# luizirber/sourmash-rust

Hardware: AMD Instinct MI355X
Metric: k-mers hashed/sec (k=31, scaled=1000) (higher is better)
Workload: dtype u64

## Files before the change

### sourmash-rust_amd/csrc/sketch_kernels.hip

```cpp
#include <hip/hip_runtime.h>
#include <stdint.h>

#include <cstdio>
#include <cstdlib>
#include <type_traits>

#include "device.hpp"
#include "kernels.hpp"

namespace smh {
namespace {

constexpr uint64_t kC1 = 0x87c37b91114253d5ULL;
constexpr uint64_t kC2 = 0x4cf5ad432745937fULL;

__device__ __forceinline__ uint64_t rotl64(uint64_t x, int r) { return (x << r) | (x >> (64 - r)); }
__device__ __forceinline__ uint64_t fmix64(uint64_t k) {
  k ^= k >> 33;
  k *= 0xff51afd7ed558ccdULL;
  k ^= k >> 33;
  k *= 0xc4ceb9fe1a85ec53ULL;
  k ^= k >> 33;
  return k;
}
// ... 20 lines not shown
    uint32_t r = n & 15u;
    if (r < 8) k1 |= (uint64_t)b << (8 * r);
    else k2 |= (uint64_t)b << (8 * (r - 8));
    n++;
    if ((n & 15u) == 0) { mm3_block(h1, h2, k1, k2); k1 = 0; k2 = 0; }
  }
  __device__ __forceinline__ uint64_t finish() {
    uint32_t rem = n & 15u;
    if (rem > 8) h2 ^= mix_k2(k2);
    if (rem > 0) h1 ^= mix_k1(k1);
    return mm3_finish(h1, h2, n);
  }
};

__device__ __forceinline__ void emit(const CandSink& sink, uint64_t h, uint64_t pos) {
  unsigned long long idx = atomicAdd(sink.count, 1ull);
  if (idx < sink.capacity) {
    sink.hash[idx] = h;
    if (sink.pos) sink.pos[idx] = pos;
  }
}

struct Stage {
  uint32_t* ctl;
  uint64_t* hash;
  uint64_t* pos;
  uint32_t cap;
};
__device__ __forceinline__ void stage_emit(const Stage& st, const CandSink& sink, uint64_t h, uint64_t pos) {
  const uint32_t slot = atomicAdd(&st.ctl[0], 1u);
  if (slot < st.cap) { st.hash[slot] = h; if (sink.pos) st.pos[slot] = pos; }
  else emit(sink, h, pos);
}
__device__ __forceinline__ void stage_flush(const Stage& st, const CandSink& sink, int tid, int nthreads,
                                            uint32_t at_least = 0) {
  __syncthreads();
  const uint32_t staged = min(st.ctl[0], st.cap);
  if (staged && staged >= at_least) {
    if (tid == 0) {
      unsigned long long base = atomicAdd(sink.count, (unsigned long long)staged);
      st.ctl[2] = (uint32_t)base; st.ctl[3] = (uint32_t)(base >> 32);
    }
    __syncthreads();
    const uint64_t base = ((uint64_t)st.ctl[3] << 32) | st.ctl[2];
    for (uint32_t e = tid; e < staged; e += nthreads)
      if (base + e < sink.capacity) {
        sink.hash[base + e] = st.hash[e];
        if (sink.pos) sink.pos[base + e] = st.pos[e];
      }
    __syncthreads();
    if (tid == 0) st.ctl[0] = 0;
  }
}

__device__ __forceinline__ uint32_t find_record(const uint64_t* __restrict__ starts, uint32_t nrec,
                                                uint64_t p) {
  uint32_t lo = 0, hi = nrec;
  while (hi - lo > 1) {
    uint32_t mid = (lo + hi) >> 1;
    if (starts[mid] <= p) lo = mid; else hi = mid;
  }
  return lo;
}

__device__ __forceinline__ uint64_t record_valid_end(const uint64_t* __restrict__ starts, const uint64_t* __restrict__ vends,
                                                     uint32_t min_len, uint32_t r) {
  if (vends) return vends[r];
  const uint64_t s0 = starts[r], s1 = starts[r + 1];
  return (min_len && s1 - s0 < min_len) ? s0 : s1;
}
__global__ __launch_bounds__(256) void k_tile_records(const uint64_t* __restrict__ starts, const uint64_t* __restrict__ vends,
                                                      uint32_t nrec, uint32_t min_len, uint64_t base, uint64_t tile,
                                                      uint64_t ntiles, TileRec* __restrict__ out) {
  const uint64_t t = (uint64_t)blockIdx.x * blockDim.x + threadIdx.x;
  if (t >= ntiles) return;
  const uint32_t r = find_record(starts, nrec, base + t * tile);
  out[t] = TileRec{r, find_record(starts, nrec, base + (t + 1) * tile), record_valid_end(starts, vends, min_len, r)};
}
__device__ __forceinline__ uint32_t find_record_in_tile(const SeqBatch& b, uint32_t min_len, uint64_t tix, uint64_t p,
                                                        uint64_t* end) {
  uint32_t lo = 0, hi = b.nrec;
  if (b.tile_rec) {
    const TileRec t = b.tile_rec[tix];
    if (t.last == t.rec) { *end = t.end; return t.rec; }
    lo = t.rec; hi = t.last + 1;
  }
  while (hi - lo > 1) {
    const uint32_t mid = (lo + hi) >> 1;
    if (b.starts[mid] <= p) lo = mid; else hi = mid;
  }
  *end = record_valid_end(b.starts, b.vends, min_len, lo);
  return lo;
}

__device__ __forceinline__ uint32_t upper(uint32_t c) { return (c >= 'a' && c <= 'z') ? c - 32 : c; }

constexpr int kLutEntries = 256 + 256 + 64 + 1;
constexpr int kLutDwords = kLutEntries * 3;
constexpr int kLutDwordsFold = kLutEntries * 5;
constexpr uint64_t kC1x2 = kC1 * 2;

struct W2 { uint32_t lo, hi; };
__device__ __forceinline__ W2 w2_rotl(W2 x, int r) {
  if (r < 32) return {__builtin_amdgcn_alignbit(x.lo, x.hi, 32 - r), __builtin_amdgcn_alignbit(x.hi, x.lo, 32 - r)};
  return {__builtin_amdgcn_alignbit(x.hi, x.lo, 64 - r), __builtin_amdgcn_alignbit(x.lo, x.hi, 64 - r)};
}
__device__ __forceinline__ W2 w2_mul(W2 x, uint64_t c) {
  const uint32_t cl = (uint32_t)c, ch = (uint32_t)(c >> 32);
  uint64_t t, u, p, cy;
  asm("v_mad_u64_u32 %0, %1, %2, %3, 0" : "=v"(t), "=s"(cy) : "v"(x.hi), "s"(cl));
  asm("v_mad_u64_u32 %0, %1, %2, %3, %4" : "=v"(u), "=s"(cy) : "v"(x.lo), "s"(ch), "v"(t));
  asm("v_mad_u64_u32 %0, %1, %2, %3, 0" : "=v"(p), "=s"(cy) : "v"(x.lo), "s"(cl));
  uint32_t hi;
  asm("v_add_u32 %0, %1, %2" : "=v"(hi) : "v"((uint32_t)(p >> 32)), "v"((uint32_t)u));
  return {(uint32_t)p, hi};
}
__device__ __forceinline__ W2 w2_xor(W2 a, W2 b) { return {a.lo ^ b.lo, a.hi ^ b.hi}; }
__device__ __forceinline__ uint64_t w2_pair(W2 a) {
  uint64_t v = ((uint64_t)a.hi << 32) | a.lo;
  asm("" : "+v"(v));
  return v;
}
__device__ __forceinline__ W2 w2_split(uint64_t v) { return {(uint32_t)v, (uint32_t)(v >> 32)}; }
__device__ __forceinline__ W2 w2_add(W2 a, W2 b) { return w2_split(w2_pair(a) + w2_pair(b)); }
__device__ __forceinline__ void w2_cross_add(W2& h1, W2& h2) {
  uint64_t a = w2_pair(h1), b = w2_pair(h2);
  a += b; b += a;
  h1 = w2_split(a); h2 = w2_split(b);
}
__device__ __forceinline__ W2 w2_mul5_add(W2 x, uint64_t c) {
  const uint64_t v = w2_pair(x);
  uint64_t t;
  asm("v_lshl_add_u64 %0, %1, 2, %1" : "=v"(t) : "v"(v));
  return w2_split(t + c);
}
__device__ __forceinline__ W2 w2_fmix_open(W2 k) {
  k.lo ^= k.hi >> 1;
  k = w2_mul(k, 0xff51afd7ed558ccdULL);
  k.lo ^= k.hi >> 1;
  k = w2_mul(k, 0xc4ceb9fe1a85ec53ULL);
  return k;
}
__device__ __forceinline__ uint32_t open_thr(uint64_t thr) {
  const uint32_t hi = (uint32_t)(thr >> 32);
  return hi == 0xffffffffu ? hi : hi + 1u;
}
__device__ __forceinline__ bool open_may_pass(W2 a, W2 b, uint32_t thr_hi1) { return a.hi + b.hi + 1u <= thr_hi1; }
__device__ __forceinline__ uint64_t open_finish(W2 a, W2 b) {
  a.lo ^= a.hi >> 1; b.lo ^= b.hi >> 1;
  return ((((uint64_t)a.hi << 32) | a.lo) + (((uint64_t)b.hi << 32) | b.lo));
}
__device__ __forceinline__ W2 w2_add_keep(W2 a, W2 b) {
  uint64_t r;
  asm("v_lshl_add_u64 %0, %1, 0, %2" : "=v"(r) : "v"(((uint64_t)a.hi << 32) | a.lo), "v"(((uint64_t)b.hi << 32) | b.lo));
  return w2_split(r);
}
constexpr uint64_t kFmixC2 = 0xc4ceb9fe1a85ec53ULL;
__device__ __forceinline__ W2 w2_fmix_pre(W2 k) {
  k.lo ^= k.hi >> 1;
  k = w2_mul(k, 0xff51afd7ed558ccdULL);
  k.lo ^= k.hi >> 1;
  return k;
}
__device__ __forceinline__ uint32_t open_hi_sum1(W2 ka, W2 kb) {
  const uint32_t cl = (uint32_t)kFmixC2, ch = (uint32_t)(kFmixC2 >> 32);
  uint64_t s0, s1, s2, s3, cy;
  asm("v_mad_u64_u32 %0, %1, %2, %3, 1" : "=v"(s0), "=s"(cy) : "v"(ka.hi), "s"(cl));
  asm("v_mad_u64_u32 %0, %1, %2, %3, %4" : "=v"(s1), "=s"(cy) : "v"(ka.lo), "s"(ch), "v"(s0));
  asm("v_mad_u64_u32 %0, %1, %2, %3, %4" : "=v"(s2), "=s"(cy) : "v"(kb.hi), "s"(cl), "v"(s1));
  asm("v_mad_u64_u32 %0, %1, %2, %3, %4" : "=v"(s3), "=s"(cy) : "v"(kb.lo), "s"(ch), "v"(s2));
  return (uint32_t)s3 + __umulhi(ka.lo, cl) + __umulhi(kb.lo, cl);
}
__device__ __forceinline__ uint64_t open_full(W2 ka, W2 kb) { return open_finish(w2_mul(ka, kFmixC2), w2_mul(kb, kFmixC2)); }
__device__ __forceinline__ W2 mix_k1_fold(uint32_t S, W2 T) {
  const uint32_t cl = (uint32_t)kC2, ch = (uint32_t)(kC2 >> 32), s1 = S >> 1;
  uint64_t p, cy;
  asm("v_mad_u64_u32 %0, %1, %2, %3, %4" : "=v"(p), "=s"(cy) : "v"(s1), "s"(cl), "v"(((uint64_t)T.hi << 32) | T.lo));
  uint32_t hi, top;
  asm("v_add_u32 %0, %1, %2" : "=v"(hi) : "v"((uint32_t)(p >> 32)), "v"(s1 * ch));
  asm("v_lshl_add_u32 %0, %1, 31, %2" : "=v"(top) : "v"(S), "v"(hi));
  return {(uint32_t)p, top};
}
__device__ __forceinline__ W2 mix_k2_fold(uint32_t S, W2 T) {
  const uint32_t cl = (uint32_t)kC1x2, ch = (uint32_t)(kC1x2 >> 32);
  uint64_t p, cy;
  asm("v_mad_u64_u32 %0, %1, %2, %3, %4" : "=v"(p), "=s"(cy) : "v"(S), "s"(cl), "v"(((uint64_t)T.hi << 32) | T.lo));
  uint32_t hi;
  asm("v_add_u32 %0, %1, %2" : "=v"(hi) : "v"((uint32_t)(p >> 32)), "v"(S * ch));
  return {(uint32_t)p, hi};
}
template <bool FOLD>
__device__ __forceinline__ W2 mix_word(int w, W2 M, uint32_t S) {
  if (FOLD) return (w & 1) ? mix_k2_fold(S, M) : mix_k1_fold(S, M);
  return (w & 1) ? w2_mul(w2_rotl(M, 33), kC1) : w2_mul(w2_rotl(M, 31), kC2);
}
template <int L, bool FOLD>
__device__ __forceinline__ void murmur_kmer_pre(const W2 (&M)[2 * L], const uint32_t (&S)[2 * L], int K, uint64_t seed, W2 seedv,
                                                W2& a, W2& b) {
  W2 h1 = seedv, h2 = seedv;
  const int nblocks = K >> 4, tail = K & 15;
#pragma unroll
  for (int blk = 0; blk < L; blk++) {
    const int w1 = 2 * blk, w2 = 2 * blk + 1;
    if (blk < nblocks) {
      h1 = w2_xor(h1, mix_word<FOLD>(w1, M[w1], S[w1]));
      if (blk == 0) h1 = w2_mul5_add(w2_rotl(h1, 27), seed * 5 + 0x52dce729u);
      else h1 = w2_mul5_add(w2_add(w2_rotl(h1, 27), h2), 0x52dce729u);
      h2 = w2_xor(h2, mix_word<FOLD>(w2, M[w2], S[w2]));
      h2 = w2_mul5_add(w2_add_keep(w2_rotl(h2, 31), h1), 0x38495ab5u);
    } else if (blk == nblocks) {
      if (tail > 8) h2 = w2_xor(h2, mix_word<FOLD>(w2, M[w2], S[w2]));
      if (tail > 0) h1 = w2_xor(h1, mix_word<FOLD>(w1, M[w1], S[w1]));
    }
  }
  h1.lo ^= (uint32_t)K; h2.lo ^= (uint32_t)K;
  w2_cross_add(h1, h2);
  a = w2_fmix_pre(h1); b = w2_fmix_pre(h2);
}

template <int KT, int THREADS, int HB, int L, bool PR = false, bool PK = false, int MINW = (PK ? 8 : 4)>
__global__ __launch_bounds__(THREADS, MINW) void k_dna_rolling(SeqBatch b, HashParams hp, CandSink sink,
                                                                     int logR, uint32_t stage_cap) {
  constexpr bool FOLD = PK && L == 2;
  __shared__ __attribute__((aligned(16))) uint32_t lut[FOLD ? kLutDwordsFold : kLutDwords];
  extern __shared__ __attribute__((aligned(16))) uint32_t smem[];
  uint32_t* st_ctl = smem;
  uint64_t* st_hash = reinterpret_cast<uint64_t*>(st_ctl + 4);
  uint64_t* st_pos = st_hash + stage_cap;
  uint32_t* tile = reinterpret_cast<uint32_t*>(st_pos + (sink.pos ? stage_cap : 0));
  const Stage stage{st_ctl, st_hash, st_pos, stage_cap};

  const int K = KT ? KT : (int)hp.ksize;
  const int tid = threadIdx.x;
  const uint32_t R = 1u << logR;
  const uint64_t TILE = (uint64_t)THREADS << logR;
  uint32_t MASK[L];
#pragma unroll
  for (int i = 0; i < L; i++) {
    const int bits = 2 * K - 32 * i;
    MASK[i] = bits >= 32 ? 0xffffffffu : (bits <= 0 ? 0u : ((1u << bits) - 1u));
  }
  const int top_limb = (2 * K - 2) >> 5, top_sh = (2 * K - 2) & 31;
  const bool multi = b.starts != nullptr;

  const int g_last = (K - 1) >> 2, nb_last = K - 4 * g_last;
  const uint64_t c_last = ((g_last >> 1) & 1) ? kC2 : kC1;
  uint64_t* ptab = reinterpret_cast<uint64_t*>(lut);
  for (int e = tid; e < kLutEntries; e += THREADS) {
    const uint32_t ent = (uint32_t)e;
    const uint32_t idx = ent & 255u;
    const int nb = ent < 512 ? 4 : (ent < 576 ? nb_last : 0);
    uint32_t v = 0;
    for (int j = 0; j < nb; j++) v |= ((0x54474341u >> (8 * ((idx >> (2 * j)) & 3))) & 0xffu) << (8 * j);
    const uint64_t c = ent < 256 ? kC1 : (ent < 512 ? kC2 : c_last);
    const uint64_t prod = (uint64_t)v * c;
    if (FOLD) {
      const uint64_t mm = (uint32_t)prod;
      const uint64_t t = c == kC1 ? (mm << 31) * kC2 : ((mm >> 31) | ((mm & 0x7fffffffu) << 33)) * kC1;
      reinterpret_cast<uint4*>(lut)[e] = make_uint4((uint32_t)t, (uint32_t)(t >> 32), (uint32_t)(prod >> 32), 0u);
      lut[4 * kLutEntries + e] = (uint32_t)prod;
    } else {
      ptab[e] = prod;
      lut[2 * kLutEntries + e] = (uint32_t)prod;
    }
  }
  uint32_t gbase[4 * L];
#pragma unroll
  for (int g = 0; g < 4 * L; g++) {
    const int nb = K - 4 * g;
    uint32_t ent0 = 576u;
    if (nb >= 4) ent0 = ((g >> 1) & 1) ? 256u : 0u;
    else if (nb > 0) ent0 = 512u;
    constexpr uint32_t esz = FOLD ? 16u : 8u;
    gbase[g] = (g & 1) ? esz * kLutEntries + ent0 * 4u : ent0 * esz;
  }
  if (tid == 0) st_ctl[0] = 0;

  const uint64_t span = hp.range_hi - hp.range_lo;
  const uint64_t ntiles = (span + TILE - 1) / TILE;
  const uintptr_t gend = ((uintptr_t)(b.seq + b.len) + 15) & ~(uintptr_t)15;
  const uint32_t nsteps = (R + (uint32_t)K - 1 + 3) & ~3u;
  const uint32_t warm_end = K > 4 ? ((uint32_t)(K - 1) & ~3u) : 0u;

  for (uint64_t tix = blockIdx.x; tix < ntiles; tix += gridDim.x) {
    const uint64_t T0 = hp.range_lo + tix * TILE;
    const uint64_t thr = hp.thr;
    const uint32_t thr_hi1 = open_thr(hp.thr);
    W2 seedv{(uint32_t)hp.seed, (uint32_t)(hp.seed >> 32)};
    asm volatile("" : "+v"(seedv.lo), "+v"(seedv.hi));
    uint64_t lthr = hp.thr;

    const uintptr_t g0 = (uintptr_t)(b.seq + T0);
    const uintptr_t ga = g0 & ~(uintptr_t)15;
    const uint32_t m = (uint32_t)(g0 - ga);
    const uint32_t nchunks = (m + (uint32_t)TILE + 16 * L + 8 + 15 + (PK ? 32u : 0u)) >> 4;
    const uint32_t nchunks_cap = (15u + (uint32_t)TILE + 16 * L + 8 + 15 + 32u) >> 4;
    __syncthreads();
    uint32_t* dirty = tile + (nchunks_cap + (nchunks_cap >> (logR - 4)) + 2);
    if (PK) {
      for (uint32_t c = tid; c < (nchunks >> 3) + 3; c += THREADS) dirty[c] = 0;
      if (tid == 0) st_ctl[1] = 0;
      __syncthreads();
    }
    for (uint32_t c = tid; c < nchunks; c += THREADS) {
      uintptr_t addr = ga + ((uintptr_t)c << 4);
      uint4 v = make_uint4(0, 0, 0, 0);
      if (addr < gend) v = *reinterpret_cast<const uint4*>(addr);
      if (PK) {
        const uint32_t w4[4] = {v.x, v.y, v.z, v.w};
        uint32_t codes = 0, bad = 0;
#pragma unroll
        for (int q = 0; q < 4; q++) {
          const uint32_t u4 = w4[q] & 0xDFDFDFDFu;
          const uint32_t c2 = (u4 >> 1) & 0x03030303u;
          const uint32_t code4 = c2 ^ ((c2 >> 1) & 0x01010101u);
          const uint32_t exp4 = __builtin_amdgcn_perm(0u, 0x54474341u, code4);
          bad |= (u4 != exp4) ? (1u << q) : 0u;
          const uint32_t pk = code4 | (code4 >> 6);
          codes |= ((pk & 0xfu) | ((pk >> 12) & 0xf0u)) << (8 * q);
        }
        tile[c + (c >> (logR - 4))] = codes;
        if (bad) { atomicOr(&dirty[c >> 3], bad << (4u * (c & 7u))); st_ctl[1] = 1; }
      } else {
        uint32_t x = c << 4;
        uint32_t o = (x >> 2) + (x >> logR);
        tile[o] = v.x; tile[o + 1] = v.y; tile[o + 2] = v.z; tile[o + 3] = v.w;
      }
    }
    __syncthreads();

    const uint64_t p0 = T0 + ((uint64_t)tid << logR);
    if (p0 < hp.range_hi) {
    const uint32_t nk = (hp.range_hi - p0) < R ? (uint32_t)(hp.range_hi - p0) : R;
    const uint32_t hi_ok = nk + (uint32_t)K - 1;

    uint32_t rec = 0;
    uint64_t cur_end = b.vend0;
    if (multi) {
      rec = find_record_in_tile(b, 0, tix, p0, &cur_end);
      if (PR) lthr = hp.thr_rec[rec];
    }
    uint32_t lim = 0;
    if (cur_end > p0) lim = (cur_end - p0) > 0xfffffffeull ? 0xffffffffu : (uint32_t)(cur_end - p0);
    uint32_t vstart = 0;
    uint32_t g_lo = 0, g_span = 0;
    uint64_t dmask = 0;
    if (PK && st_ctl[1]) {
      const uint32_t b0 = (m + ((uint32_t)tid << logR)) >> 2;
      const uint32_t* dw = reinterpret_cast<const uint32_t*>(tile) + (nchunks_cap + (nchunks_cap >> (logR - 4)) + 2);
      const uint32_t i = b0 >> 5, sft = b0 & 31u;
      const uint64_t lo64 = ((uint64_t)dw[i + 1] << 32) | dw[i];
      const uint32_t d2 = dw[i + 2];
      dmask = (lo64 >> sft) | (sft ? ((uint64_t)d2 << (64 - sft)) : 0ull);
      if (m & 3u) dmask |= (dmask >> 1) | ((uint64_t)((d2 >> sft) & 1u) << 63);
    }
    auto set_clean_window = [&](bool warm, uint32_t from_i) {
      uint32_t lim2 = warm ? lim : (lim < hi_ok ? lim : hi_ok);
      if (PK) {
        const uint32_t g = from_i >> 2;
        const uint64_t rem = g < 64 ? (dmask >> g) : 0ull;
        if (rem) lim2 = min(lim2, (g + (uint32_t)__builtin_ctzll(rem)) * 4u);
      }
      g_lo = warm ? vstart : vstart + (uint32_t)K - 1;
      g_span = lim2 >= g_lo + 4 ? lim2 - 3 - g_lo : 0u;
    };

    const uint32_t xu = m & ~3u;
    uint32_t ta = xu + ((uint32_t)tid << logR);
    ta = ta + ((ta >> logR) << 2);
    const uint32_t sh = m & 3u;
    uint32_t cur = PK ? 0u : tile[ta >> 2];
    uint32_t cq = (m >> 4) + ((uint32_t)tid << (logR - 4));
    const uint32_t sh2 = (m & 15u) * 2u;
    uint32_t pcur = PK ? tile[cq + (cq >> (logR - 4))] : 0u, w = 0, wc = 0;
    uint32_t cf[L], fle[L];
#pragma unroll
    for (int i = 0; i < L; i++) { cf[i] = 0; fle[i] = 0; }
    constexpr bool kRoll31 = PK && L == 2 && KT == 31;
    uint32_t fa0 = 0, fa1 = 0, cs0 = 0, cs1 = 0, wr = 0;

    auto group = [&](uint32_t i0, auto hashing) {
      constexpr bool kHash = decltype(hashing)::value;
      uint32_t code4 = 0, ccode4 = 0, diff4 = 0;
      if (PK) {
        if ((i0 & 12u) == 0) {
          cq += 1;
          const uint32_t pnxt = tile[cq + (cq >> (logR - 4))];
          w = __builtin_amdgcn_alignbit(pnxt, pcur, sh2);
          pcur = pnxt;
          wc = ~w;
          if (kRoll31) {
            fa1 |= w << 30;
            const uint32_t r = __builtin_bitreverse32(w);
            wr = ~(((r >> 1) & 0x55555555u) | ((r << 1) & 0xaaaaaaaau));
          }
        }
      } else {
        const uint32_t xn = xu + i0 + 4;
        ta += (xn & (R - 1)) == 0 ? 8u : 4u;
        const uint32_t nxt = tile[ta >> 2];
        const uint32_t d = __builtin_amdgcn_alignbyte(nxt, cur, sh);
        cur = nxt;
        const uint32_t u4 = d & 0xDFDFDFDFu;
        const uint32_t c2 = (u4 >> 1) & 0x03030303u;
        code4 = c2 ^ ((c2 >> 1) & 0x01010101u);
        const uint32_t exp4 = __builtin_amdgcn_perm(0u, 0x54474341u, code4);
        diff4 = u4 ^ exp4;
        ccode4 = code4 ^ 0x03030303u;
      }
      uint32_t okmask = 0xFu;
      uint64_t tq[4];
      if (PR) { tq[0] = lthr; tq[1] = lthr; tq[2] = lthr; tq[3] = lthr; }
      if (!((PK || diff4 == 0) && i0 - g_lo < g_span)) {
        if (PK && i0 < 256u && ((dmask >> (i0 >> 2)) & 1ull)) {
          uint32_t d = 0;
#pragma unroll
          for (int q = 0; q < 4; q++) {
            const uint64_t at = p0 + i0 + (uint32_t)q;
            if (at < b.len) d |= (uint32_t)b.seq[at] << (8 * q);
          }
          const uint32_t u4 = d & 0xDFDFDFDFu;
          const uint32_t c2 = (u4 >> 1) & 0x03030303u;
          const uint32_t cd = c2 ^ ((c2 >> 1) & 0x01010101u);
          diff4 = u4 ^ __builtin_amdgcn_perm(0u, 0x54474341u, cd);
        }
        okmask = 0;
#pragma unroll
        for (int q = 0; q < 4; q++) {
          const uint32_t i = i0 + q;
          uint32_t bad = (diff4 >> (8 * q)) & 0xffu;
          if (i >= lim) {
            const uint64_t qpos = p0 + i;
            if (multi) {
              while (rec + 1 < b.nrec && qpos >= b.starts[rec + 1]) { rec++; vstart = i; }
              cur_end = b.vends ? b.vends[rec] : b.starts[rec + 1];
              if (PR) lthr = hp.thr_rec[rec];
            }
            if (qpos >= cur_end) { bad = 1; lim = i + 1; }
            else lim = (cur_end - p0) > 0xfffffffeull ? 0xffffffffu : (uint32_t)(cur_end - p0);
          }
          if (bad) vstart = i + 1;
          if (kHash) {
            const bool ok = (i + 1 >= vstart + (uint32_t)K) && (i < hi_ok);
            okmask |= ok ? (1u << q) : 0u;
            if (PR) tq[q] = lthr;
          }
        }
        set_clean_window(!kHash, i0 + 4);
      }
#pragma unroll
      for (int g0b = 0; g0b < 4; g0b += HB) {
        uint32_t X[HB][L];
#pragma unroll
        for (int q = 0; q < HB; q++) {
          const int bb = g0b + q;
          const uint32_t code = PK ? (w >> (2 * bb)) & 3u : (code4 >> (8 * bb)) & 3u;
          const uint32_t ccode = PK ? (wc >> (2 * bb)) & 3u : (ccode4 >> (8 * bb)) & 3u;
          if (kRoll31) {
            const uint32_t fhu = __builtin_amdgcn_alignbit(w >> 2, fa1, 2 * bb + 2);
            fle[0] = __builtin_amdgcn_alignbit(fa1, fa0, 2 * bb + 2);
            fle[L - 1] = fhu & MASK[L - 1];
            cf[0] = __builtin_amdgcn_alignbit(cs0, wr, 30 - 2 * bb);
            cf[L - 1] = __builtin_amdgcn_alignbit(cs1, cs0, 30 - 2 * bb) & MASK[L - 1];
            if (bb == 3) { fa0 = fle[0]; fa1 = fhu; cs0 = cf[0]; cs1 = cf[L - 1]; }
          } else {
#pragma unroll
          for (int li = L - 1; li > 0; li--) cf[li] = __builtin_amdgcn_alignbit(cf[li], cf[li - 1], 30) & MASK[li];
          cf[0] = ((cf[0] << 2) | ccode) & MASK[0];
#pragma unroll
          for (int li = 0; li < L - 1; li++) fle[li] = __builtin_amdgcn_alignbit(fle[li + 1], fle[li], 2);
          fle[L - 1] >>= 2;
#pragma unroll
          for (int li = 0; li < L; li++)
            if (li == top_limb) fle[li] |= code << top_sh;
          }
          if (kHash) {
            bool fwd = false;
            if (L == 2) {
              fwd = (((uint64_t)fle[1] << 32) | fle[0]) < (((uint64_t)cf[1] << 32) | cf[0]);
            } else {
              bool decided = false;
#pragma unroll
              for (int li = L - 1; li >= 0; li--) {
                const uint32_t f = fle[li], r = cf[li];
                if (!decided && f != r) { fwd = f < r; decided = true; }
              }
            }
#pragma unroll
            for (int li = 0; li < L; li++) X[q][li] = fwd ? fle[li] : cf[li];
          }
        }
        if (kHash && i0 + g0b + HB >= (uint32_t)K && i0 + g0b < R + (uint32_t)K - 1) {
          W2 ha[HB], hb[HB];
#pragma unroll
          for (int q = 0; q < HB; q++) {
            W2 M[2 * L];
            uint32_t S[2 * L];
#pragma unroll
            for (int wi = 0; wi < 2 * L; wi++) { M[wi] = W2{0u, 0u}; S[wi] = 0u; }
#pragma unroll
            for (int g = 0; g < 4 * L; g++) {
              if (KT == 0 || 4 * g < K) {
                const uint32_t xw = X[q][g >> 2];
                uint32_t off;
                if ((g & 3) == 0 && FOLD) asm("v_lshlrev_b32_sdwa %0, 4, %1 dst_sel:DWORD dst_unused:UNUSED_PAD src0_sel:DWORD src1_sel:BYTE_0" : "=v"(off) : "v"(xw));
                else if ((g & 3) == 0) asm("v_lshlrev_b32_sdwa %0, 3, %1 dst_sel:DWORD dst_unused:UNUSED_PAD src0_sel:DWORD src1_sel:BYTE_0" : "=v"(off) : "v"(xw));
                else if ((g & 3) == 1) asm("v_lshlrev_b32_sdwa %0, 2, %1 dst_sel:DWORD dst_unused:UNUSED_PAD src0_sel:DWORD src1_sel:BYTE_1" : "=v"(off) : "v"(xw));
                else if ((g & 3) == 2 && FOLD) asm("v_lshlrev_b32_sdwa %0, 4, %1 dst_sel:DWORD dst_unused:UNUSED_PAD src0_sel:DWORD src1_sel:BYTE_2" : "=v"(off) : "v"(xw));
                else if ((g & 3) == 2) asm("v_lshlrev_b32_sdwa %0, 3, %1 dst_sel:DWORD dst_unused:UNUSED_PAD src0_sel:DWORD src1_sel:BYTE_2" : "=v"(off) : "v"(xw));
                else asm("v_lshlrev_b32_sdwa %0, 2, %1 dst_sel:DWORD dst_unused:UNUSED_PAD src0_sel:DWORD src1_sel:BYTE_3" : "=v"(off) : "v"(xw));
                const char* at = reinterpret_cast<const char*>(lut) + gbase[g] + off;
                if ((g & 1) == 0 && FOLD) {
                  typedef uint32_t u32x4 __attribute__((ext_vector_type(4)));
                  u32x4 e = *reinterpret_cast<const u32x4*>(at);
                  asm("" : "+v"(e));
                  M[g >> 1] = W2{e.x, e.y};
                  S[g >> 1] = e.z;
                } else if ((g & 1) == 0) {
                  const uint2 e = *reinterpret_cast<const uint2*>(at);
                  M[g >> 1] = W2{e.x, e.y};
                } else if (FOLD) {
                  S[g >> 1] += *reinterpret_cast<const uint32_t*>(at);
                } else {
                  M[g >> 1].hi += *reinterpret_cast<const uint32_t*>(at);
                }
              }
            }
            murmur_kmer_pre<L, FOLD>(M, S, K, hp.seed, seedv, ha[q], hb[q]);
          }
#pragma unroll
          for (int q = 0; q < HB; q++)
            if (open_hi_sum1(ha[q], hb[q]) <= (PR ? open_thr(tq[g0b + q]) : thr_hi1)) {
              uint32_t om = okmask;
              asm volatile("" : "+v"(om));
              const uint64_t h = open_full(ha[q], hb[q]);
              if (h <= (PR ? tq[g0b + q] : thr) && ((om >> (g0b + q)) & 1u))
                stage_emit(stage, sink, h, hp.pos_base + p0 + (i0 + g0b + q + 1 - (uint32_t)K));
            }
        }
      }
      if (PK) { w >>= 8; wc >>= 8; }
      if (kRoll31) wr <<= 8;
    };

    set_clean_window(true, 0);
    uint32_t i0 = 0;
    for (; i0 < warm_end; i0 += 4) group(i0, std::false_type{});
    set_clean_window(false, i0);
    for (; i0 < nsteps; i0 += 4) group(i0, std::true_type{});
    }

    stage_flush(stage, sink, tid, THREADS);
  }
}

__global__ __launch_bounds__(256) void k_dna_generic(SeqBatch b, HashParams hp, CandSink sink) {
  const uint64_t K = hp.ksize;
  const uint64_t stride = (uint64_t)gridDim.x * blockDim.x;
  for (uint64_t p = hp.range_lo + (uint64_t)blockIdx.x * blockDim.x + threadIdx.x; p < hp.range_hi;
       p += stride) {
    uint64_t end = b.vend0, thr = hp.thr;
    if (b.starts) {
      uint32_t r = find_record(b.starts, b.nrec, p);
      end = b.vends ? b.vends[r] : b.starts[r + 1];
      if (hp.thr_rec) thr = hp.thr_rec[r];
    }
    if (p + K > end || p + K < p) continue;
    const uint8_t* s = b.seq + p;
    bool ok = true, decided = false, fwd = true;
    for (uint64_t i = 0; i < K; i++) {
      uint32_t f = upper(s[i]);
      if (!(f == 'A' || f == 'C' || f == 'G' || f == 'T')) { ok = false; break; }
      if (!decided) {
        uint32_t t = upper(s[K - 1 - i]);
        uint32_t rc = t == 'A' ? 'T' : t == 'T' ? 'A' : t == 'C' ? 'G' : t == 'G' ? 'C' : t;
        if (f != rc) { fwd = f < rc; decided = true; }
      }
    }
    if (!ok) continue;
    Mm3Stream st(hp.seed);
    for (uint64_t i = 0; i < K; i++) {
      uint32_t c;
      if (fwd) c = upper(s[i]);
      else {
        uint32_t t = upper(s[K - 1 - i]);
        c = t == 'A' ? 'T' : t == 'T' ? 'A' : t == 'C' ? 'G' : 'C';
      }
      st.push(c);
    }
    uint64_t h = st.finish();
    if (h <= thr) emit(sink, h, hp.pos_base + p);
  }
}

__global__ __launch_bounds__(256) void k_first_invalid(SeqBatch b, uint64_t* __restrict__ vends) {
  const uintptr_t p0 = (uintptr_t)b.seq, pa = p0 & ~(uintptr_t)15;
  const uint64_t head = p0 - pa;
  const uint64_t nch = (head + b.len + 15) >> 4;
  const uint64_t stride = (uint64_t)gridDim.x * blockDim.x;
  for (uint64_t c = (uint64_t)blockIdx.x * blockDim.x + threadIdx.x; c < nch; c += stride) {
    const uint4 v = *reinterpret_cast<const uint4*>(pa + (c << 4));
    const uint32_t w[4] = {v.x, v.y, v.z, v.w};
#pragma unroll
    for (int k = 0; k < 4; k++) {
      const uint32_t u4 = w[k] & 0xDFDFDFDFu;
      const uint32_t c2 = (u4 >> 1) & 0x03030303u;
      const uint32_t code4 = c2 ^ ((c2 >> 1) & 0x01010101u);
      const uint32_t diff4 = u4 ^ __builtin_amdgcn_perm(0u, 0x54474341u, code4);
      if (diff4 == 0) continue;
      for (int j = 0; j < 4; j++) {
        if (((diff4 >> (8 * j)) & 0xffu) == 0) continue;
        const uint64_t at = (c << 4) + 4 * k + j;
        if (at < head || at - head >= b.len) continue;
        const uint64_t q = at - head;
        const uint32_t r = b.starts ? find_record(b.starts, b.nrec, q) : 0;
        atomicMin((unsigned long long*)&vends[r], (unsigned long long)q);
      }
    }
  }
}
__global__ __launch_bounds__(256) void k_first_bad_record(const uint64_t* __restrict__ starts, const uint64_t* __restrict__ vends,
                                                          uint32_t nrec, uint32_t ksize, unsigned long long* __restrict__ out) {
  unsigned long long best = ~0ull;
  for (uint64_t r = (uint64_t)blockIdx.x * blockDim.x + threadIdx.x; r < nrec; r += (uint64_t)gridDim.x * blockDim.x) {
    const uint64_t st = starts[r], en = starts[r + 1];
    if (vends[r] < en && en - st >= ksize && r < best) best = r;
  }
  for (int off = 32; off; off >>= 1) {
    const unsigned long long o = __shfl_down(best, off);
    best = o < best ? o : best;
  }
  if ((threadIdx.x & 63) == 0 && best != ~0ull) atomicMin(out, best);
}

constexpr uint32_t kDropped = 0xFFu;
__constant__ char kCodonAA[65] =
    "FFLLSSSSYY**CC*W" "LLLLPPPPHHQQRRRR" "IIIMTTTTNNKKSSRR" "VVVVAAAADDEEGGGG";

__device__ __forceinline__ int tcag(uint32_t c) {
  return c == 'T' ? 0 : c == 'C' ? 1 : c == 'A' ? 2 : c == 'G' ? 3 : -1;
}
__device__ __forceinline__ uint32_t comp_upper(uint32_t c) {
  return c == 'A' ? 'T' : c == 'T' ? 'A' : c == 'C' ? 'G' : c == 'G' ? 'C' : c;
}
__device__ __forceinline__ bool utf8_ok3(uint32_t a, uint32_t c, uint32_t d) {
  auto cont = [](uint32_t v) { return v >= 0x80 && v <= 0xBF; };
  auto lead2 = [](uint32_t v) { return v >= 0xC2 && v <= 0xDF; };
  if (a < 0x80) {
    if (c < 0x80) return d < 0x80;
    return lead2(c) && cont(d);
  }
  if (lead2(a)) return cont(c) && d < 0x80;
  if (a == 0xE0) return c >= 0xA0 && c <= 0xBF && cont(d);
  if (a == 0xED) return c >= 0x80 && c <= 0x9F && cont(d);
  if (a >= 0xE1 && a <= 0xEF) return cont(c) && cont(d);
  return false;
}

constexpr int kTrThreads = 256;
constexpr int kTrPerThread = 12;
constexpr int kTrTile = kTrThreads * kTrPerThread;

__global__ __launch_bounds__(kTrThreads) void k_translate(SeqBatch b, const uint64_t* __restrict__ seg_off,
                                                          uint32_t nseg, uint32_t ksize, uint8_t* __restrict__ res,
                                                          uint32_t* __restrict__ bad_utf8) {
  __shared__ __attribute__((aligned(16))) uint8_t tile[kTrTile + 64];
  __shared__ __attribute__((aligned(16))) uint8_t code[kTrTile + 64];
  __shared__ uint8_t lut_code[256];
  __shared__ uint8_t lut_aa[64];
  const int tid = threadIdx.x;
  {
    const uint32_t c = (uint32_t)tid, u = upper(c);
    const int t = tcag(u);
    lut_code[tid] = t < 0 ? 0x80u : (uint8_t)t;
    if (tid < 64) lut_aa[tid] = (uint8_t)kCodonAA[tid];
  }
  const uint64_t ntiles = (b.len + kTrTile - 1) / kTrTile;
  const uintptr_t gend = ((uintptr_t)(b.seq + b.len) + 15) & ~(uintptr_t)15;
  const uint64_t per_wg = (ntiles + gridDim.x - 1) / gridDim.x;
  const uint64_t t_begin = (uint64_t)blockIdx.x * per_wg;
  const uint64_t t_end = t_begin + per_wg < ntiles ? t_begin + per_wg : ntiles;
  uint32_t rec0 = 0;
  if (b.starts && t_begin < t_end) rec0 = find_record(b.starts, b.nrec, t_begin * kTrTile);
  for (uint64_t tix = t_begin; tix < t_end; tix++) {
    const uint64_t T0 = tix * kTrTile;
    if (b.starts)
      while (rec0 + 1 < b.nrec && T0 >= b.starts[rec0 + 1]) rec0++;
    const uintptr_t g0 = (uintptr_t)(b.seq + T0);
    const uintptr_t ga = (g0 & ~(uintptr_t)15) - 16;
    const uint32_t m = (uint32_t)(g0 - ga);
    __syncthreads();
    for (uint32_t c = tid; c < (kTrTile + 64) / 16; c += kTrThreads) {
      const uintptr_t addr = ga + ((uintptr_t)c << 4);
      uint4 v = make_uint4(0, 0, 0, 0);
      if (addr >= ((uintptr_t)b.seq & ~(uintptr_t)15) && addr < gend) v = *reinterpret_cast<const uint4*>(addr);
      *reinterpret_cast<uint4*>(tile + (c << 4)) = v;
      uint32_t w[4] = {v.x, v.y, v.z, v.w}, o[4];
#pragma unroll
      for (int d = 0; d < 4; d++)
        o[d] = (uint32_t)lut_code[w[d] & 0xff] | ((uint32_t)lut_code[(w[d] >> 8) & 0xff] << 8) |
               ((uint32_t)lut_code[(w[d] >> 16) & 0xff] << 16) | ((uint32_t)lut_code[w[d] >> 24] << 24);
      *reinterpret_cast<uint4*>(code + (c << 4)) = make_uint4(o[0], o[1], o[2], o[3]);
    }
    __syncthreads();
    uint32_t rec = 0;
    uint64_t rs = 0, re = b.len;
    const uint64_t pfirst = T0 + (uint64_t)tid * kTrPerThread;
    if (b.starts && pfirst < b.len) {
      rec = rec0;
      if (rec0 + 8 < b.nrec && pfirst >= b.starts[rec0 + 8]) rec = find_record(b.starts, b.nrec, pfirst);
      rs = b.starts[rec]; re = b.starts[rec + 1];
    }
    bool packed = false;
    if (pfirst < b.len) {
      while (pfirst >= re) { rec++; rs = b.starts[rec]; re = b.starts[rec + 1]; }
      const uint64_t rl = re - rs, o = pfirst - rs;
      packed = rl >= ksize && o >= 2 && o + kTrPerThread + 2 <= rl;
      if (packed) {
        const uint32_t x0 = m + (uint32_t)(pfirst - T0);
        uint32_t k[kTrPerThread + 4];
        uint32_t anybad = 0;
#pragma unroll
        for (int i = 0; i < kTrPerThread + 4; i++) { k[i] = code[x0 - 2 + i]; anybad |= k[i]; }
        if (anybad & 0x80u) packed = false;
        if (packed) {
          const uint32_t of = (uint32_t)(o % 3);
          const uint64_t back0 = rl - 1 - o;
          const uint32_t bf = (uint32_t)(back0 % 3);
#pragma unroll
          for (int c = 0; c < 3; c++) {
            uint32_t v = 0;
#pragma unroll
            for (int t = 0; t < 4; t++) {
              const int i = 2 + c + 3 * t;
              v |= (uint32_t)lut_aa[(k[i] << 4) | (k[i + 1] << 2) | k[i + 2]] << (8 * t);
            }
            uint32_t fr = of + c; fr = fr >= 3 ? fr - 3 : fr;
            __builtin_memcpy(res + seg_off[6 * rec + 2 * fr] + (o + c) / 3, &v, 4);
            uint32_t w = 0;
#pragma unroll
            for (int t = 0; t < 4; t++) {
              const int i = 2 + c + 3 * t;
              w |= (uint32_t)lut_aa[((k[i] << 4) | (k[i - 1] << 2) | k[i - 2]) ^ 0x2a] << (8 * (3 - t));
            }
            uint32_t br = bf + 3 - c; br = br >= 3 ? br - 3 : br;
            __builtin_memcpy(res + seg_off[6 * rec + 2 * br + 1] + (back0 - c) / 3 - 3, &w, 4);
          }
        }
      }
    }
    if (!packed) {
    for (int q = 0; q < kTrPerThread; q++) {
      const uint64_t p = pfirst + q;
      if (p >= b.len) break;
      while (p >= re) { rec++; rs = b.starts[rec]; re = b.starts[rec + 1]; }
      const uint64_t rl = re - rs, o = p - rs;
      if (rl < ksize) continue;
      const uint32_t x = m + (uint32_t)(p - T0);
      const uint32_t k0 = code[x];
      if (o + 2 < rl) {
        const uint32_t k1 = code[x + 1], k2 = code[x + 2];
        const uint32_t seg = 6 * rec + 2 * (uint32_t)(o % 3);
        const uint32_t bad = (k0 | k1 | k2) & 0x80u;
        if (bad) {
          const uint32_t c0 = upper(tile[x]), c1 = upper(tile[x + 1]), c2 = upper(tile[x + 2]);
          if (((c0 | c1 | c2) & 0x80u) && !utf8_ok3(c0, c1, c2)) atomicOr(&bad_utf8[seg], 1u);
        }
        res[seg_off[seg] + o / 3] = bad ? (uint8_t)kDropped : lut_aa[(k0 << 4) | (k1 << 2) | k2];
      }
      if (o >= 2) {
        const uint32_t k1 = code[x - 1], k2 = code[x - 2];
        const uint64_t back = rl - 1 - o;
        const uint32_t seg = 6 * rec + 2 * (uint32_t)(back % 3) + 1;
        const uint32_t bad = (k0 | k1 | k2) & 0x80u;
        if (bad) {
          const uint32_t d0 = comp_upper(upper(tile[x])), d1 = comp_upper(upper(tile[x - 1])), d2 = comp_upper(upper(tile[x - 2]));
          if (((d0 | d1 | d2) & 0x80u) && !utf8_ok3(d0, d1, d2)) atomicOr(&bad_utf8[seg], 1u);
        }
        res[seg_off[seg] + back / 3] = bad ? (uint8_t)kDropped : lut_aa[(((k0 << 4) | (k1 << 2) | k2)) ^ 0x2a];
      }
    }
    }
  }
}


__global__ __launch_bounds__(256) void k_protein_positions(uint64_t* __restrict__ pos, const unsigned long long* __restrict__ count,
                                                           uint64_t capacity, const uint64_t* __restrict__ starts, uint32_t nrec,
                                                           uint64_t batch_len, const uint64_t* __restrict__ seg_off, uint32_t kb,
                                                           uint64_t pos_base) {
  const uint64_t n = *count < capacity ? *count : capacity;
  const uint64_t stride = (uint64_t)gridDim.x * blockDim.x;
  for (uint64_t i = (uint64_t)blockIdx.x * blockDim.x + threadIdx.x; i < n; i += stride) {
    const uint64_t code = pos[i], a = code >> 1;
    uint32_t rec = 0;
    uint64_t rs = 0, re = batch_len;
    if (starts) { rec = find_record(starts, nrec, a); rs = starts[rec]; re = starts[rec + 1]; }
    const uint64_t a_rel = a - rs, len = re - rs;
    uint64_t g;
    if ((code & 1) == 0) {
      g = seg_off[6 * (uint64_t)rec + 2 * (a_rel % 3)] + a_rel / 3;
    } else {
      const uint64_t rcidx = len - a_rel - kb;
      g = seg_off[6 * (uint64_t)rec + 2 * (rcidx % 3) + 1] + rcidx / 3;
    }
    pos[i] = pos_base + g;
  }
}

__device__ __forceinline__ int dna_digit(uint32_t c) {
  const uint32_t u = c & 0xDFu;
  return u == 'A' ? 0 : u == 'C' ? 1 : u == 'G' ? 2 : u == 'T' ? 3 : -1;
}
__device__ __forceinline__ uint32_t aa_of_digits(int d0, int d1, int d2) {
  const int t[4] = {2, 1, 3, 0};
  return (uint32_t)(uint8_t)kCodonAA[16 * t[d0] + 4 * t[d1] + t[d2]];
}

__device__ __forceinline__ void spliced_windows(const SeqBatch& b, const HashParams& hp, const CandSink& sink, uint32_t win, uint64_t a) {
  const uint32_t kb = 3 * win;
  uint32_t rec = 0;
  uint64_t rs = 0, re = b.len;
  if (b.starts) { rec = find_record(b.starts, b.nrec, a); rs = b.starts[rec]; re = b.starts[rec + 1]; }
  const uint64_t len = re - rs;
  if (len < hp.ksize || a < rs || a >= re) return;
  {
    const uint32_t f = (uint32_t)((a - rs) % 3);
    const uint64_t fend = rs + f + 3 * ((len - f) / 3);
    Mm3Stream st(hp.seed);
    uint32_t got = 0;
    for (uint64_t c = a; c + 3 <= fend && got < win; c += 3) {
      const int d0 = dna_digit(b.seq[c]), d1 = dna_digit(b.seq[c + 1]), d2 = dna_digit(b.seq[c + 2]);
      if (d0 < 0 || d1 < 0 || d2 < 0) { if (c == a) break; continue; }
      st.push(aa_of_digits(d0, d1, d2));
      got++;
    }
    if (got == win) {
      const uint64_t h = st.finish();
      if (h <= hp.thr) emit(sink, h, a << 1);
    }
  }
  if (a + kb <= re) {
    const uint64_t e = a + kb - 1;
    Mm3Stream st(hp.seed);
    uint32_t got = 0;
    for (uint64_t c = e; c >= rs + 2 && got < win; c -= 3) {
      const int d0 = dna_digit(b.seq[c]), d1 = dna_digit(b.seq[c - 1]), d2 = dna_digit(b.seq[c - 2]);
      if (d0 < 0 || d1 < 0 || d2 < 0) { if (c == e) break; if (c < 3) break; continue; }
      st.push(aa_of_digits(3 - d0, 3 - d1, 3 - d2));
      got++;
      if (c < 3) break;
    }
// ... 656 lines not shown
```

Measured before the change: 400.6 billion.

## Replace per-group warm-up with direct rolling-state init and cheaper 2-bit packing

For the k=31 packed rolling path, the warm-up loop over the first groups is replaced by building the forward, reverse-complement and window state straight from two packed tile words with bit-reverse and alignbit. The tile-fill packing now encodes bases with a single udot4 plus a gray-code fix-up. It builds per-chunk bad flags only when some byte mismatches, by reloading the chunk. The clean-window bounds also let full, record-aligned windows skip the k-1 edge offset when k-1 divides the hash batch. This removes warm-up hashing work and per-chunk ALU work, but adds intricate bit manipulation with correctness risk at record and dirty boundaries.

```diff
diff --git a/sourmash-rust_amd/csrc/sketch_kernels.hip b/sourmash-rust_amd/csrc/sketch_kernels.hip
--- a/sourmash-rust_amd/csrc/sketch_kernels.hip
+++ b/sourmash-rust_amd/csrc/sketch_kernels.hip
@@ -346,25 +346,35 @@
       if (tid == 0) st_ctl[1] = 0;
       __syncthreads();
     }
+    const uint64_t cin64 = gend > ga ? (uint64_t)(gend - ga) >> 4 : 0ull;
+    const uint32_t cin = cin64 < nchunks ? (uint32_t)cin64 : nchunks;
+    uint32_t kActg;
+    asm("s_mov_b32 %0, 0x47544341" : "=s"(kActg));
     for (uint32_t c = tid; c < nchunks; c += THREADS) {
-      uintptr_t addr = ga + ((uintptr_t)c << 4);
       uint4 v = make_uint4(0, 0, 0, 0);
-      if (addr < gend) v = *reinterpret_cast<const uint4*>(addr);
+      if (c < cin) v = *reinterpret_cast<const uint4*>(ga + ((uintptr_t)c << 4));
       if (PK) {
         const uint32_t w4[4] = {v.x, v.y, v.z, v.w};
-        uint32_t codes = 0, bad = 0;
+        uint32_t xany = 0, gray = 0;
 #pragma unroll
         for (int q = 0; q < 4; q++) {
           const uint32_t u4 = w4[q] & 0xDFDFDFDFu;
-          const uint32_t c2 = (u4 >> 1) & 0x03030303u;
-          const uint32_t code4 = c2 ^ ((c2 >> 1) & 0x01010101u);
-          const uint32_t exp4 = __builtin_amdgcn_perm(0u, 0x54474341u, code4);
-          bad |= (u4 != exp4) ? (1u << q) : 0u;
-          const uint32_t pk = code4 | (code4 >> 6);
-          codes |= ((pk & 0xfu) | ((pk >> 12) & 0xf0u)) << (8 * q);
-        }
-        tile[c + (c >> (logR - 4))] = codes;
-        if (bad) { atomicOr(&dirty[c >> 3], bad << (4u * (c & 7u))); st_ctl[1] = 1; }
+          const uint32_t g4 = (u4 >> 1) & 0x03030303u;
+          xany |= u4 ^ __builtin_amdgcn_perm(0u, kActg, g4);
+          gray |= __builtin_amdgcn_udot4(g4, 0x40100401u, 0u, false) << (8 * q);
+        }
+        tile[c + (c >> (logR - 4))] = gray ^ ((gray >> 1) & 0x55555555u);
+        if (xany) {
+          const volatile uint32_t* src = reinterpret_cast<const volatile uint32_t*>(ga + ((uintptr_t)c << 4));
+          uint32_t bad = 0;
+#pragma unroll
+          for (int q = 0; q < 4; q++) {
+            const uint32_t u4 = (c < cin ? src[q] : 0u) & 0xDFDFDFDFu;
+            bad |= u4 != __builtin_amdgcn_perm(0u, kActg, (u4 >> 1) & 0x03030303u) ? 1u << q : 0u;
+          }
+          atomicOr(&dirty[c >> 3], bad << (4u * (c & 7u)));
+          st_ctl[1] = 1;
+        }
       } else {
         uint32_t x = c << 4;
         uint32_t o = (x >> 2) + (x >> logR);
@@ -398,14 +408,16 @@
       dmask = (lo64 >> sft) | (sft ? ((uint64_t)d2 << (64 - sft)) : 0ull);
       if (m & 3u) dmask |= (dmask >> 1) | ((uint64_t)((d2 >> sft) & 1u) << 63);
     }
+    constexpr bool kEdgeFree = KT > 0 && (KT - 1) % HB == 0;
     auto set_clean_window = [&](bool warm, uint32_t from_i) {
-      uint32_t lim2 = warm ? lim : (lim < hi_ok ? lim : hi_ok);
+      const bool whole = warm || (kEdgeFree && vstart == 0 && nk == R);
+      uint32_t lim2 = whole ? lim : (lim < hi_ok ? lim : hi_ok);
       if (PK) {
         const uint32_t g = from_i >> 2;
         const uint64_t rem = g < 64 ? (dmask >> g) : 0ull;
         if (rem) lim2 = min(lim2, (g + (uint32_t)__builtin_ctzll(rem)) * 4u);
       }
-      g_lo = warm ? vstart : vstart + (uint32_t)K - 1;
+      g_lo = whole ? vstart : vstart + (uint32_t)K - 1;
       g_span = lim2 >= g_lo + 4 ? lim2 - 3 - g_lo : 0u;
     };
 
@@ -464,9 +476,9 @@
             if (at < b.len) d |= (uint32_t)b.seq[at] << (8 * q);
           }
           const uint32_t u4 = d & 0xDFDFDFDFu;
-          const uint32_t c2 = (u4 >> 1) & 0x03030303u;
-          const uint32_t cd = c2 ^ ((c2 >> 1) & 0x01010101u);
-          diff4 = u4 ^ __builtin_amdgcn_perm(0u, 0x54474341u, cd);
+          uint32_t actg;
+          asm("s_mov_b32 %0, 0x47544341" : "=s"(actg));
+          diff4 = u4 ^ __builtin_amdgcn_perm(0u, actg, (u4 >> 1) & 0x03030303u);
         }
         okmask = 0;
 #pragma unroll
@@ -588,10 +600,23 @@
     };
 
     set_clean_window(true, 0);
-    uint32_t i0 = 0;
-    for (; i0 < warm_end; i0 += 4) group(i0, std::false_type{});
-    set_clean_window(false, i0);
-    for (; i0 < nsteps; i0 += 4) group(i0, std::true_type{});
+    if (kRoll31 && !PR && g_span > 24u) {
+      const uint32_t d1 = tile[cq + 1 + ((cq + 1) >> (logR - 4))], d2 = tile[cq + 2 + ((cq + 2) >> (logR - 4))];
+      const uint32_t q0 = __builtin_amdgcn_alignbit(d1, pcur, sh2), q1 = __builtin_amdgcn_alignbit(d2, d1, sh2);
+      cq += 2; pcur = d2;
+      fa0 = q0 << 6;
+      fa1 = __builtin_amdgcn_alignbit(q1, q0, 26);
+      const uint32_t r0 = __builtin_bitreverse32(q0), r1 = __builtin_bitreverse32(q1);
+      const uint32_t c0 = ~(((r0 >> 1) & 0x55555555u) | ((r0 << 1) & 0xaaaaaaaau));
+      const uint32_t c1 = ~(((r1 >> 1) & 0x55555555u) | ((r1 << 1) & 0xaaaaaaaau));
+      cs0 = __builtin_amdgcn_alignbit(c0, c1, 8);
+      cs1 = c0 >> 8;
+      w = q1 >> 24; wc = ~q1 >> 24; wr = c1 << 24;
+    } else {
+      for (uint32_t i0 = 0; i0 < warm_end; i0 += 4) group(i0, std::false_type{});
+    }
+    set_clean_window(false, warm_end);
+    for (uint32_t i0 = warm_end; i0 < nsteps; i0 += 4) group(i0, std::true_type{});
     }
 
     stage_flush(stage, sink, tid, THREADS);
```

Measured after the change: 412.7 billion (median of 6 runs). +3.0%, better.
